# ratt-ru/pfb-clean

Hardware: AMD Instinct MI355X
Metric: PCG matvecs/sec (FFT-conv A^H A apply), 4k x 4k x 8-band cube (higher is better)
Workload: dtype f32; 1 GPU; 4096x4096x8-band cube PCG (hessian_psf + Tikhonov, M = x/sigmainv, tol=0, minit=maxit=20); nx_psf=8192, bands_per_gpu=8, parallelism=band-shard x1, allreduce_hook=False

## Files before the change

include/pfb_hip.h:

```cpp
#ifndef PFB_HIP_H
#define PFB_HIP_H

#include <stddef.h>
#include <stdint.h>

#ifdef __cplusplus
extern "C" {
#endif

#define PFB_ABI_VERSION 1

#define PFB_F32 0
#define PFB_F64 1

#define PFB_OK               0
#define PFB_ERR_INVALID     -1
#define PFB_ERR_UNSUPPORTED -2
#define PFB_ERR_HIP         -3
#define PFB_ERR_NONFINITE   -4
#define PFB_ERR_ALLOC       -5
#define PFB_ERR_COMM        -6

#define PFB_PCG_CONVERGED     0
#define PFB_PCG_MAXIT         1
// ... 22 lines not shown
                      const void* x, const void* beam, double wsum, double sigmainv,
                      void* out, const void* dot_with, double* dot_out, void* stream);

int pfb_psfconv_apply_dots(pfb_conv_plan* plan, int band0, int nb,
                           const void* x, const void* beam, double wsum, double sigmainv,
                           void* out, const void* dot_with, const void* dot_with2,
                           double* dots_out, void* stream);

int pfb_psfconv_apply_dots_bands(pfb_conv_plan* plan, int band0, int nb,
                                 const void* x, const void* beam, double wsum, double sigmainv,
                                 void* out, const void* dot_with, const void* dot_with2,
                                 double* dots_out, void* stream);

int    pfb_psfconv_plan_info(const pfb_conv_plan* plan, int* fast_path, int* vb,
                             size_t* workspace_bytes);

int pfb_psfconv_set_profiling(pfb_conv_plan* plan, int on);
int pfb_psfconv_get_profile(pfb_conv_plan* plan, double stage_ms[3], int* napply);

#define PFB_REDUCE_WS_DOUBLES 8192

int pfb_dot(int dtype, const void* a, const void* b, size_t n,
            double* out, double* ws, void* stream);
int pfb_norm_diff_sums(int dtype, const void* x, const void* xp, size_t n,
                       double* out, double* ws, void* stream);
int pfb_any_nonzero(int dtype, const void* a, size_t n, double* out, double* ws,
                    void* stream);
int pfb_axpby(int dtype, double a, const void* x, double b, void* y, size_t n,
              void* stream);

// ... 162 lines not shown
```

pfb_clean_amd/_lib.py:

```python
import ctypes as C
import os

_HERE = os.path.dirname(os.path.abspath(__file__))
LIB_PATH = os.environ.get('PFB_HIP_LIB') or os.path.join(_HERE, 'libpfb_hip.so')

PFB_F32, PFB_F64 = 0, 1
PFB_OK = 0
ERRORS = {-1: 'invalid argument', -2: 'unsupported size/dtype', -3: 'HIP runtime error',
          -4: 'non-finite value', -5: 'device allocation failed', -6: 'band-shard exchange failed'}
PCG_STATUS = {0: 'converged', 1: 'maxit', 2: 'zero-residual', 3: 'breakdown'}
REDUCE_WS_DOUBLES = 8192


PFB_ERR_INVALID = -1
PFB_ERR_UNSUPPORTED = -2
PFB_ERR_ALLOC = -5
PFB_ERR_COMM = -6


class PfbHipError(RuntimeError):
    def __init__(self, code, msg):
        super().__init__(f"libpfb_hip: {ERRORS.get(code, code)}: {msg}")
        self.code = code

# ... 12 lines not shown

_vp, _i, _d, _sz = C.c_void_p, C.c_int, C.c_double, C.c_size_t
SIGNATURES = {
    'pfb_abi_version': (_i, []),
    'pfb_last_error': (C.c_char_p, []),
    'pfb_psfconv_plan_create': (_i, [_i, _i, _i, _i, _i, _i, C.POINTER(_vp)]),
    'pfb_psfconv_plan_destroy': (_i, [_vp]),
    'pfb_psfconv_set_psfhat': (_i, [_vp, _vp, _vp]),
    'pfb_psfconv_apply': (_i, [_vp, _i, _i, _vp, _vp, _d, _d, _vp, _vp, _vp, _vp]),
    'pfb_psfconv_set_psf': (_i, [_vp, _vp, _vp, _vp]),
    'pfb_psfhat_regrid': (_i, [_i, _vp, _i, _i, _i, _i, _i, _i, _i, _vp, _vp]),
    'pfb_psfhat_from_psf': (_i, [_i, _vp, _i, _i, _i, _vp, _vp]),
    'pfb_psfconv_apply_dots': (_i, [_vp, _i, _i, _vp, _vp, _d, _d, _vp, _vp, _vp, _vp, _vp]),
    'pfb_psfconv_apply_dots_bands': (_i, [_vp, _i, _i, _vp, _vp, _d, _d, _vp, _vp, _vp, _vp, _vp]),
    'pfb_psfconv_plan_info': (_i, [_vp, C.POINTER(_i), C.POINTER(_i), C.POINTER(_sz)]),
    'pfb_psfconv_set_profiling': (_i, [_vp, _i]),
    'pfb_psfconv_get_profile': (_i, [_vp, C.POINTER(_d), C.POINTER(_i)]),
    'pfb_dot': (_i, [_i, _vp, _vp, _sz, _vp, _vp, _vp]),
    'pfb_norm_diff_sums': (_i, [_i, _vp, _vp, _sz, _vp, _vp, _vp]),
    'pfb_any_nonzero': (_i, [_i, _vp, _sz, _vp, _vp, _vp]),
    'pfb_axpby': (_i, [_i, _d, _vp, _d, _vp, _sz, _vp]),
    'pfb_pcg_work_bytes': (_sz, [_vp, _i]),
    'pfb_pcg_solve': (_i, [_vp, _i, _i, _vp, _vp, _vp, _vp, _d, _d, _d, _d, _i, _i, _i,
                           _vp, ALLREDUCE_FN, _vp, C.POINTER(PcgResult), _vp]),
    'pfb_pcg_bands_work_bytes': (_sz, [_vp, _i]),
    'pfb_pcg_solve_bands': (_i, [_vp, _i, _i, _vp, _vp, _vp, _vp, _d, _d, _d, _d, _i, _i, _i,
                                 _vp, C.POINTER(PcgResult), _vp]),
    'pfb_bandmix_dots': (_i, [_i, _vp, _vp, _i, _sz, _d, _vp, _vp, _vp, _vp, _vp, _vp]),
    'pfb_hessparam_work_bytes': (_sz, [_vp]),
    'pfb_hessparam_apply': (_i, [_vp, _vp, _vp, _vp, _d, _vp, _vp, _vp, _vp]),
# ... 78 lines not shown
```

pfb_clean_amd/csrc/cgvec.hip:

```cpp
#include "conv_plan.hpp"
#include "pcg_state.hpp"
#include <chrono>
#include <unistd.h>
#include <cstring>
#include <cstdlib>
#include <utility>
#include <vector>

namespace pfb {

constexpr int RED_MAX_GRID = 1024;

static inline int red_grid(size_t nvec) {
    size_t g = (nvec + RED_BLOCK - 1) / RED_BLOCK;
    g = (g + 3) / 4;
    if (g < 1) g = 1;
    if (g > (size_t)RED_MAX_GRID) g = RED_MAX_GRID;
    return (int)g;
}

template <typename T, int V>
__global__ void __launch_bounds__(RED_BLOCK)
k_dot(const T* __restrict__ a, const T* __restrict__ b, size_t nvec, double* __restrict__ ws) {
    double acc[1] = {0.0};
// ... 139 lines not shown
    for (size_t i = (size_t)blockIdx.x * blockDim.x + threadIdx.x; i < nvec;
         i += (size_t)gridDim.x * blockDim.x) {
        Pack<T, V> pp = ld<T, V>(p, i), pr = ld<T, V>(r, i);
#pragma unroll
        for (int e = 0; e < V; ++e) {
            const T y = mdiv > T(0) ? pr.e[e] / mdiv : pr.e[e];
            const T v = beta * pp.e[e] - y;
            pp.e[e] = v;
            acc[0] += (v != T(0)) ? 1.0 : 0.0;
        }
        st<T, V>(p, i, pp);
    }
    emit_partials<1>(acc, ws);
}

template <typename T, int V, int U, bool XNT, bool REV>
__global__ void __launch_bounds__(RED_BLOCK)
k_pcg_update_dir(const T* x, const T* r, T* __restrict__ p, const T* __restrict__ Ap, T* xn, T* rn,
                 const double* __restrict__ S, T mdiv, size_t nvs, int gps, double* __restrict__ ws) {
    const int s = blockIdx.x / gps, g = blockIdx.x - s * gps;
    const double* Sb = S + (size_t)s * SB;
    { const size_t off = (size_t)s * nvs * V; x += off; r += off; p += off; Ap += off; xn += off; rn += off; }
    double acc[4] = {0.0, 0.0, 0.0, 0.0};
    if (sys_live(Sb)) {
        const T alpha = (T)Sb[S_ALPHA];
        const T beta = (T)Sb[S_BETA];
        const size_t stride = (size_t)gps * blockDim.x;
        for (size_t i0 = (size_t)g * blockDim.x + threadIdx.x; i0 < nvs; i0 += U * stride) {
            Pack<T, V> px[U], pr[U], pp[U], pa[U];
#pragma unroll
            for (int u = 0; u < U; ++u) {
                const size_t ii = i0 + u * stride;
                const size_t i = REV ? nvs - 1 - ii : ii;
                if (ii < nvs) {
                    px[u] = XNT ? ld_nt<T, V>(x, i) : ld<T, V>(x, i);
                    pr[u] = ld<T, V>(r, i); pp[u] = ld<T, V>(p, i); pa[u] = ld<T, V>(Ap, i);
                }
            }
#pragma unroll
            for (int u = 0; u < U; ++u) {
                const size_t ii = i0 + u * stride;
                const size_t i = REV ? nvs - 1 - ii : ii;
                if (ii >= nvs) break;
                Pack<T, V> ox, orr;
#pragma unroll
                for (int e = 0; e < V; ++e) {
                    const T xnew = px[u].e[e] + alpha * pp[u].e[e];
                    const T rnew = pr[u].e[e] + alpha * pa[u].e[e];
                    const T y = mdiv > T(0) ? rnew / mdiv : rnew;
                    ox.e[e] = xnew;
                    orr.e[e] = rnew;
                    const double d = (double)xnew - (double)px[u].e[e];
                    acc[0] += (double)rnew * (double)y;
                    acc[1] += d * d;
                    acc[2] += (double)xnew * (double)xnew;
                    const T pn = beta * pp[u].e[e] - y;
                    pp[u].e[e] = pn;
                    acc[3] += (pn != T(0)) ? 1.0 : 0.0;
                }
                if constexpr (XNT) st_nt<T, V>(xn, i, ox); else st<T, V>(xn, i, ox);
                st<T, V>(rn, i, orr);
                st<T, V>(p, i, pp[u]);
            }
        }
    } else if (xn != x) {
        for (size_t i = (size_t)g * blockDim.x + threadIdx.x; i < nvs; i += (size_t)gps * blockDim.x) {
            st<T, V>(xn, i, ld<T, V>(x, i));
            st<T, V>(rn, i, ld<T, V>(r, i));
        }
    }
    emit_partials<4>(acc, ws);
}

__global__ void k_set_alpha(double* S) { S[S_ALPHA] = S[S_RHO] / S[S_PAP]; S[S_NBT] = 0.0; }
__global__ void k_scale_alpha(double* S) { S[S_ALPHA] *= 0.75; }
__global__ void k_set_beta(double* S) { S[S_BETA] = S[S_RHON] / S[S_RHO]; }
// ... 334 lines not shown
            return false;
        };
        int err;
        bool lookahead = n <= lookahead_max;
        if (const char* la = getenv("PFB_PCG_LOOKAHEAD")) lookahead = atoi(la) != 0;
        if (lookahead && plan->pcg_pin_n < nsys) {
            if (plan->pcg_pin) { PFB_HIP_CHECK(hipStreamSynchronize(st)); (void)hipHostFree(plan->pcg_pin); }
            plan->pcg_pin = nullptr;
            plan->pcg_pin_n = 0;
            PFB_HIP_CHECK(hipHostMalloc((void**)&plan->pcg_pin, sizeof(double) * 2 * nS, hipHostMallocDefault));
            plan->pcg_pin_n = nsys;
            for (int e = 0; e < 2; ++e)
                if (!plan->pcg_ev[e]) PFB_HIP_CHECK(hipEventCreateWithFlags(&plan->pcg_ev[e], hipEventDisableTiming));
        }
        const bool xnt = vec && n * sizeof(T) >= ((size_t)32 << 20);
        const double* seen = h.data();
        bool go = (1.0 > tol || 0 < minit) && 0 < maxit && any_live(seen);
        int khost = 0, slot = 0;
        bool pending_end = false, have_prev = false;
        int lo = 0, nl = nsys, gpl = update_grid(nvs, nsys);
        T *xc = x, *rc = r, *xn = xalt ? xalt : x, *rn = ralt ? ralt : r;
        auto narrow = [&](const double* hs) {
            int a = 0, z = nsys;
            while (a < z && !sys_live(hs + (size_t)a * SB)) ++a;
            while (z > a && !sys_live(hs + (size_t)(z - 1) * SB)) --z;
            if (z > a && (a != lo || z - a != nl)) { lo = a; nl = z - a; gpl = update_grid(nvs, nl); }
        };
        while (go) {
            const size_t off = (size_t)lo * ns;
            double* Sl = S + (size_t)lo * SB;
            typename PcgOp<T>::Partials c;
            if ((err = A.apply_partials(p, Ap, rc, lo, nl, &c)) != PFB_OK) return err;
            hipLaunchKernelGGL(k_iter_sums, dim3(nl), dim3(256), 0, st, c.cp, c.bs, c.qs, c.bst,
                               (const double*)ws, gpl, pending_end ? 1 : 0, Sl, mdiv_d, predict, hook ? 0 : 1);
            if (hook) {
                if ((err = sync.reduce(Sl + S_PAP, pending_end ? 7 : 4)) != PFB_OK) return err;
                if (pending_end) hipLaunchKernelGGL(k_iter_end_begin, dim3(1), dim3(1), 0, st, Sl, mdiv_d, predict);
                else hipLaunchKernelGGL(k_iter_begin, dim3(1), dim3(1), 0, st, Sl, mdiv_d, predict);
            }
            pending_end = false;
#define PFB_UPDATE(VV, XN)                                                                                     \
            hipLaunchKernelGGL((k_pcg_update_dir<T, VV, 2, XN, XN>), dim3(nl * gpl), dim3(RED_BLOCK), 0, st,   \
                               (const T*)xc + off, (const T*)rc + off, p + off, (const T*)Ap + off, xn + off,    \
                               rn + off, (const double*)Sl, mdiv, nvs, gpl, ws)
            if (xnt) PFB_UPDATE(V16<T>::N, true);
            else if (vec) PFB_UPDATE(V16<T>::N, false);
            else PFB_UPDATE(1, false);
#undef PFB_UPDATE
            std::swap(xc, xn);
            std::swap(rc, rn);
            if (khost + 1 < minit && khost + 1 < maxit) {
                pending_end = true;
            } else {
                if (hook) {
                    hipLaunchKernelGGL(k_iter_sums, dim3(nl), dim3(256), 0, st, (const double*)nullptr, 0, 0, 0,
                                       (const double*)ws, gpl, 1, Sl, mdiv_d, predict, 0);
                    if ((err = sync.reduce(Sl + S_RHON, 3)) != PFB_OK) return err;
                }
                hipLaunchKernelGGL(k_iter_end, dim3(nl), dim3(256), 0, st, hook ? nullptr : (const double*)ws, gpl, Sl);
            }
            PFB_HIP_CHECK(hipGetLastError());
            ++khost;
// ... 196 lines not shown
```

pfb_clean_amd/csrc/conv_plan.hpp:

```cpp
#pragma once
#include "common.hpp"
#include "fft_generic.hpp"

struct pfb_partial_layout {
    int slots, band_slots, q_stride, band_stride;
};

struct pfb_conv_plan {
    int nx, ny, P, Q, M;
    int nband, dtype;
    int VB, nvb;
    int fast;
    int long_lines;
    void* long_ws;
    size_t long_ws_bytes;
    pfb::FftFactors frow;
    pfb::FftFactors fcol;
    void* twP;
    void* twQ;
    void* psf_l;
    void* T;
    double* partials;
    size_t T_elems_per_band;
    size_t psf_elems_per_band;
    size_t workspace_bytes;
    int have_psf;
    int partials_per_band;
    pfb_partial_layout last;
    void* fast_tables;
    int prof_on, prof_n, prof_tick;
    hipEvent_t* prof_ev;
    double* pcg_pin;
    int pcg_pin_n;
    hipEvent_t pcg_ev[2];
};

namespace pfb {
inline size_t vec_bytes(const pfb_conv_plan* plan, int nb) {
    const size_t b = (size_t)nb * plan->nx * plan->ny * (plan->dtype == PFB_F32 ? 4 : 8);
    return (b + 255) & ~(size_t)255;
}
constexpr int PROF_MAX = 512;
inline void prof_mark(pfb_conv_plan* p, hipStream_t st, int k) {
    if (!p->prof_on) return;
// ... 23 lines not shown
```

pfb_clean_amd/csrc/fftconv.hip:

```cpp
#include "conv_plan.hpp"
#include "fft_long.hpp"
#include <algorithm>
#include <vector>
#include <cstring>
#include <cstdlib>

namespace pfb {

thread_local char g_err[512] = "";
void set_error(const char* fmt, ...) {
    va_list ap;
    va_start(ap, fmt);
    vsnprintf(g_err, sizeof(g_err), fmt, ap);
    va_end(ap);
}

struct ConvDims {
    int nx, ny, P, Q, M;
    size_t T_band, psf_band;
};

__device__ __forceinline__ size_t t_index(const ConvDims& d, int band, int i, int v) {
    return (size_t)band * d.T_band + (size_t)v * d.nx + i;
}
// ... 347 lines not shown
                            pfb_conv_plan** plan) {
    PFB_REQUIRE(plan != nullptr, PFB_ERR_INVALID, "plan_create: null plan pointer");
    *plan = nullptr;
    PFB_REQUIRE(dtype == PFB_F32 || dtype == PFB_F64, PFB_ERR_INVALID, "plan_create: bad dtype %d", dtype);
    PFB_REQUIRE(nx > 0 && ny > 0 && nband > 0, PFB_ERR_INVALID, "plan_create: non-positive size");
    PFB_REQUIRE(nx <= nx_psf && ny <= ny_psf, PFB_ERR_INVALID,
                "plan_create: image (%d,%d) larger than psf grid (%d,%d)", nx, ny, nx_psf, ny_psf);
    PFB_REQUIRE(ny_psf % 2 == 0, PFB_ERR_UNSUPPORTED,
                "plan_create: ny_psf=%d must be even (pfb's grid worker makes it so)", ny_psf);
    PFB_REQUIRE(factorable(nx_psf) && factorable(ny_psf / 2), PFB_ERR_UNSUPPORTED,
                "plan_create: (%d,%d) has a prime factor > 13", nx_psf, ny_psf);
    pfb_conv_plan* p = (pfb_conv_plan*)calloc(1, sizeof(pfb_conv_plan));
    PFB_REQUIRE(p != nullptr, PFB_ERR_ALLOC, "plan_create: host alloc failed");
    p->nx = nx; p->ny = ny; p->P = nx_psf; p->Q = ny_psf; p->M = ny_psf / 2;
    p->nband = nband; p->dtype = dtype;
    const size_t csz = dtype == PFB_F32 ? 8 : 16;
    p->fast = pow2_supported(p) ? 1 : 0;
    if (const char* e = getenv("PFB_FORCE_GENERIC")) { if (atoi(e)) p->fast = 0; }
    int vb = 1;
    p->partials_per_band = p->fast ? nx / pow2_rows_per_wg(p) : nx;
    if (p->fast) {
        vb = pow2_nvb(p);
        p->nvb = pow2_nblocks(p);
    } else {
        p->nvb = (p->M + 1 + vb - 1) / vb;
    }
    p->VB = vb;
    p->T_elems_per_band = (size_t)p->nvb * nx * vb;
    p->psf_elems_per_band = (size_t)p->nvb * p->P * vb;
    if (!plan_factors(p->M, &p->frow) || !plan_factors(p->P, &p->fcol)) {
// ... 40 lines not shown
    if (p->prof_ev) {
        for (int k = 0; k < 4 * PROF_MAX; ++k) (void)hipEventDestroy(p->prof_ev[k]);
        free(p->prof_ev);
    }
    if (p->pcg_pin) (void)hipHostFree(p->pcg_pin);
    for (int e = 0; e < 2; ++e) if (p->pcg_ev[e]) (void)hipEventDestroy(p->pcg_ev[e]);
    free(p);
    return PFB_OK;
}

int pfb_psfconv_plan_info(const pfb_conv_plan* p, int* fast_path, int* vb, size_t* workspace_bytes) {
    PFB_REQUIRE(p != nullptr, PFB_ERR_INVALID, "plan_info: null plan");
    if (fast_path) *fast_path = p->fast;
    if (vb) *vb = p->VB;
    if (workspace_bytes) *workspace_bytes = p->workspace_bytes;
    return PFB_OK;
}

int pfb_psfconv_set_profiling(pfb_conv_plan* p, int on) {
    PFB_REQUIRE(p != nullptr, PFB_ERR_INVALID, "set_profiling: null plan");
    if (on && !p->prof_ev) {
        p->prof_ev = (hipEvent_t*)calloc(4 * PROF_MAX, sizeof(hipEvent_t));
        PFB_REQUIRE(p->prof_ev != nullptr, PFB_ERR_ALLOC, "set_profiling: host alloc failed");
        for (int k = 0; k < 4 * PROF_MAX; ++k) PFB_HIP_CHECK(hipEventCreate(&p->prof_ev[k]));
    }
    p->prof_on = on > 0 ? on : 0;
    p->prof_n = 0;
    p->prof_tick = 0;
    return PFB_OK;
}
// ... 164 lines not shown
```

pfb_clean_amd/csrc/fftconv_pow2.hip:

```cpp
#include "conv_plan.hpp"
#include "fft_pow2.hpp"
#include <vector>
#include <cstdlib>
#include <type_traits>

#ifndef PFB_POW2_PART
#define PFB_POW2_PART 0
#endif
#define PFB_POW2_COL  (PFB_POW2_PART == 0 || PFB_POW2_PART == 2)
#define PFB_POW2_REST (PFB_POW2_PART == 0 || PFB_POW2_PART == 1)
#define PFB_POW2_MIX  (PFB_POW2_PART == 0 || PFB_POW2_PART == 3)
#define PFB_POW2_COLK  (PFB_POW2_COL || PFB_POW2_MIX)
#define PFB_POW2_RESTK (PFB_POW2_REST || PFB_POW2_MIX)

namespace pfb {

#ifndef PFB_STAMP
#define PFB_STAMP 0
#endif
#if PFB_STAMP
#define PFB_STAMP_ITS 4
#define PFB_STAMP_FIRST 2
static __device__ unsigned long long* g_stamp_buf = nullptr;
#define STAMP(KID, it, slot)                                                                              \
// ... 53 lines not shown
    return *reinterpret_cast<const Blk<T, NVB>*>(src);
}
template <typename T, int NVB>
__device__ __forceinline__ Blk<T, NVB> loadb_nt(const cplx<T>* src) {
    typedef float v4f __attribute__((ext_vector_type(4)));
    static_assert(sizeof(Blk<T, NVB>) == 16, "16-byte blocks");
    const v4f v = __builtin_nontemporal_load(reinterpret_cast<const v4f*>(src));
    Blk<T, NVB> b;
    __builtin_memcpy(&b, &v, 16);
    return b;
}

template <typename T, int NVB>
__device__ __forceinline__ void storeb(cplx<T>* dst, const Blk<T, NVB>& b) {
    *reinterpret_cast<Blk<T, NVB>*>(dst) = b;
}

template <typename P>
__device__ __forceinline__ P* opaque(P* p) {
    asm volatile("" : "+v"(p));
    return p;
}

__device__ __forceinline__ int launder(int v) {
    asm volatile("" : "+v"(v));
    return v;
}

template <typename T>
__device__ __forceinline__ cplx<T> root32(int k) {
// ... 741 lines not shown
    }
    __device__ __forceinline__ static int tile_row(int rg, int tiles_per_band) {
        constexpr int SH = 8 / G;
        if constexpr (SH > 1) {
            if (tiles_per_band % (8 * SH) == 0) {
                const int q = rg / (8 * SH), rem = rg % (8 * SH);
                rg = SH * (q * 8 + (rem & 7)) + (rem >> 3);
            }
        }
        return rg * G;
    }
};

template <typename T, int L, int PAR, typename Hook>
__device__ __forceinline__ void fwdp_post_lin(const cplx<T>* zr, const cplx<T>* ltm, cplx<T> wq1,
                                              cplx<T>* __restrict__ Tb, int nx, int i0, int rr, int bi, const Hook& hook);
template <typename T, int L, int PAR, typename Hook = NoPassHook>
__device__ __forceinline__ void fwdp_post(const cplx<T>* zr, const cplx<T>* ltm, cplx<T> wq1,
                                          cplx<T>* __restrict__ Tb, int nx, int i0, int rr, int bi,
                                          const Hook& hook = Hook()) {
    fwdp_post_lin<T, L, PAR, Hook>(zr, ltm, wq1, Tb, nx, i0, rr, bi, hook);
}

template <typename T, int L, int PAR, int K, int NREG, typename Hook>
__device__ __forceinline__ void post_steps_lin(const cplx<T>* const (&za)[FastCfg<T>::NVB], const cplx<T>* const (&zb)[FastCfg<T>::NVB],
                                               const cplx<T>* lw, cplx<T> wq1, cplx<T>* ub, size_t ustep, unsigned voff,
                                               bool first0, const Hook& hook) {
    using P = FwdP<T, L>;
    using F = typename P::F;
    constexpr int NVB = P::NVB, MS = NVB * P::BSTEP;
    if constexpr (K < NREG) {
        hook(PassIdx<K>{});
        Blk<T, NVB> o;
#pragma unroll
        for (int h = 0; h < NVB; ++h) {
            cplx<T> w;
            if constexpr (P::SMT) w = K == 0 ? lw[h] : lw[h] * root32<T>(P::KR * K);
            else w = lw[MS * K + h];
            if (PAR) w = w * wq1;
            const cplx<T> zv = za[h][F::cpad(MS * K)];
            cplx<T> zm = zb[h][F::cpad(MS * (NREG - 1 - K))];
            if constexpr (PAR == 0 && K == 0) { if (first0 && h == 0) zm = zv; }
            o.c[h] = T(0.5) * addrot<false>(addc(zv, zm), w * subc(zv, zm));
        }
        storeb<T, NVB>(ub + (size_t)K * ustep + voff, o);
        __builtin_amdgcn_sched_barrier(0);
        post_steps_lin<T, L, PAR, K + 1, NREG, Hook>(za, zb, lw, wq1, ub, ustep, voff, first0, hook);
    }
}

template <typename T, int L, int PAR, typename Hook>
__device__ __forceinline__ void fwdp_post_lin(const cplx<T>* zr, const cplx<T>* ltm, cplx<T> wq1,
                                              cplx<T>* __restrict__ Tb, int nx, int i0, int rr, int bi,
                                              const Hook& hook) {
    using P = FwdP<T, L>;
    using F = typename P::F;
    constexpr int NVB = P::NVB, BS = P::BSTEP, MS = NVB * BS;
    constexpr int NBP = PAR ? P::NBO : P::NBE;
    constexpr int NIT = (NBP + BS - 1) / BS;
    constexpr int NREG = PAR ? NIT : NIT - 1;
    static_assert(MS % 16 == 0, "a step keeps the padding phase");
    static_assert(PAR ? (NBP == NIT * BS) : (NBP == (NIT - 1) * BS + 1), "block counts of the two sweeps");
    cplx<T>* ub = Tb + (size_t)(PAR ? P::NBE : 0) * nx * NVB;
    const size_t ustep = (size_t)BS * nx * NVB;
    const unsigned voff = ((unsigned)bi * (unsigned)nx + (unsigned)(i0 + rr)) * NVB;
    const int m0 = NVB * bi;
    const cplx<T>* za[NVB];
    const cplx<T>* zb[NVB];
#pragma unroll
    for (int h = 0; h < NVB; ++h) {
        za[h] = zr + F::pad(m0 + h);
        zb[h] = zr + F::pad(L - PAR - (m0 + h) - MS * (NREG - 1));
    }
    post_steps_lin<T, L, PAR, 0, NREG, Hook>(za, zb, ltm + m0, wq1, ub, ustep, voff, bi == 0, hook);
    if constexpr (PAR == 0) {
        hook(PassIdx<NREG>{});
        const cplx<T> z0 = zr[F::pad(0)];
        Blk<T, NVB> o;
        o.c[0] = T(0.5) * addrot<false>(addc(z0, z0), cplx<T>(T(-1), T(0)) * subc(z0, z0));
#pragma unroll
        for (int h = 1; h < NVB; ++h) o.c[h] = cplx<T>(0, 0);
        storeb<T, NVB>(ub + (size_t)(NBP - 1) * nx * NVB + (unsigned)(i0 + rr) * NVB, o);
        __builtin_amdgcn_sched_barrier(0);
    }
}

template <typename T, int L, bool BEAM>
__global__ void __launch_bounds__((FwdP<T, L>::NT))
k_row_fwd_pow2q(const T* __restrict__ x, const T* __restrict__ beam, cplx<T>* __restrict__ Tw, const cplx<T>* __restrict__ twM,
                const cplx<T>* __restrict__ ptwc, FastDims d, int band0, int tiles_per_band, int ntiles,
                cplx<T> wq1) {
    using P = FwdP<T, L>;
    constexpr int E = P::EOK;
    using F = RegFft<T, L, E, false, 0, true, false>;
    constexpr int TPB = F::TPB, G = P::G, NT = P::NT, NP = F::NPASS;
    using V2 = typename vec2<T>::type;
    extern __shared__ __attribute__((aligned(16))) char smem[];
    cplx<T>* ltw = reinterpret_cast<cplx<T>*>(smem);
    cplx<T>* ltm = ltw + P::PTWP;
    cplx<T>* lds0 = ltm + P::NTM;
    int vb = blockIdx.x;
    if (vb >= ntiles) return;
    for (int k = threadIdx.x; k < F::PTWC; k += NT) ltw[k] = ptwc[k];
    for (int k = threadIdx.x; k < P::NTM; k += NT) ltm[k] = twM[k];
    V2 xa[E], ba[BEAM ? E : 1];
    {
        const int bl = vb / tiles_per_band, i0 = P::tile_row(vb - bl * tiles_per_band, tiles_per_band);
        const int g = threadIdx.x / TPB, t = threadIdx.x % TPB;
        const size_t off = (size_t)bl * d.xband + (size_t)(i0 + g) * d.xpitch;
        const V2* xr = reinterpret_cast<const V2*>(x + off) + t;
#pragma unroll
        for (int j = 0; j < E; ++j) xa[j] = xr[TPB * j];
        if constexpr (BEAM) {
            const V2* br = reinterpret_cast<const V2*>(beam + off) + t;
#pragma unroll
            for (int j = 0; j < E; ++j) ba[j] = br[TPB * j];
        }
    }
    __syncthreads();
    for (int sit = 0;; ++sit) {
        STAMP(0, sit, 0);
        const int vbn = vb + (int)gridDim.x < ntiles ? vb + (int)gridDim.x : vb;
        const int bl = vb / tiles_per_band, i0 = P::tile_row(vb - bl * tiles_per_band, tiles_per_band);
        cplx<T>* Tb = Tw + (size_t)(band0 + bl) * d.T_band;
        cplx<T> vv[E];
        {
            const int tid = launder((int)threadIdx.x);
            const int g = tid / TPB, t = tid % TPB;
            cplx<T>* lds = lds0 + (size_t)g * P::STRIDE;
#pragma unroll
            for (int j = 0; j < E; ++j) {
                if constexpr (BEAM) { xa[j].x *= ba[j].x; xa[j].y *= ba[j].y; }
                vv[j] = cplx<T>(xa[j].x, xa[j].y);
            }
            STAMP(0, sit, 1);
            F::template run<false>(vv, lds, t, ltw);
            STAMP(0, sit, 2);
        }
        {
            const int tid = launder((int)threadIdx.x);
            const int g = tid / TPB, t = tid % TPB;
            __syncthreads();
            cplx<T>* wp = lds0 + (size_t)g * P::STRIDE + F::pad(t);
#pragma unroll
            for (int j = 0; j < E; ++j) wp[F::cpad(TPB * j)] = vv[j];
            __syncthreads();
        }
        STAMP(0, sit, 3);
        {
            const int tid = launder((int)threadIdx.x);
            fwdp_post<T, L, 0>(lds0 + (size_t)(tid % G) * P::STRIDE, ltm, wq1, Tb, d.nx, i0, tid % G, tid / G);
        }
        STAMP(0, sit, 4);
        {
            const int tid = launder((int)threadIdx.x);
            const int g = tid / TPB, t = tid % TPB;
            cplx<T>* lds = lds0 + (size_t)g * P::STRIDE;
#pragma unroll
            for (int j = 0; j < E; ++j) {
                vv[j] = cplx<T>(xa[j].x, xa[j].y) * P::tw_row(ltm, t, j);
                if ((j & 3) == 3) __builtin_amdgcn_sched_barrier(0);
            }
            const int bln = vbn / tiles_per_band, i0n = P::tile_row(vbn - bln * tiles_per_band, tiles_per_band);
            const size_t offn = (size_t)bln * d.xband + (size_t)(i0n + g) * d.xpitch;
            const V2* xr = reinterpret_cast<const V2*>(x + offn) + t;
            const V2* br = BEAM ? reinterpret_cast<const V2*>(beam + offn) + t : nullptr;
            F::template run<false>(vv, lds, t, ltw, [&](auto k) {
                constexpr int K = decltype(k)::value;
#pragma unroll
                for (int j = (K * E) / NP; j < ((K + 1) * E) / NP; ++j) {
                    xa[j] = xr[TPB * j];
                    if constexpr (BEAM) ba[j] = br[TPB * j];
                }
            });
            STAMP(0, sit, 5);
        }
        {
            const int tid = launder((int)threadIdx.x);
            const int g = tid / TPB, t = tid % TPB;
            cplx<T>* wp = lds0 + (size_t)g * P::STRIDE + F::pad(t);
            __syncthreads();
#pragma unroll
            for (int j = 0; j < E; ++j) wp[F::cpad(TPB * j)] = vv[j];
            __syncthreads();
            fwdp_post<T, L, 1>(lds0 + (size_t)(tid % G) * P::STRIDE, ltm, wq1, Tb, d.nx, i0, tid % G, tid / G);
            STAMP(0, sit, 6);
            __syncthreads();
        }
        STAMP(0, sit, 7);
        if (vbn == vb) break;
        vb = vbn;
    }
}

template <typename T, int L, int E, int PAR, typename PF>
__device__ __forceinline__ void row_inv_phase(PF&& after_loads_issued, const cplx<T>* __restrict__ Tb,
                                              const cplx<T>* __restrict__ twQ,
                                              const cplx<T>* __restrict__ ptw, cplx<T>* lds0,
                                              cplx<T>* lds, int nx, int i0, int t,
                                              cplx<T> (&vv)[E]) {
// ... 752 lines not shown
}
#endif

#if PFB_POW2_RESTK
template <typename T, int L> constexpr bool fwdp_ok() {
    if constexpr (odd_part(L) > 1) return false;
    else return FwdP<T, L>::OK;
}
template <typename T, int L> struct RowFwdK {
    using FP = FwdP<T, L>;
    static constexpr bool PERSISTENT = fwdp_ok<T, L>();
    static constexpr int E = [] { if constexpr (PERSISTENT) return FP::EOK; else return RowCfg<T, L, false>::E; }();
    static constexpr auto plain() { return k_row_fwd_pow2<T, L, E>; }
    template <typename Fn> static void reachable(Fn&& f) {
        if constexpr (PERSISTENT) {
            f(k_row_fwd_pow2q<T, L, false>, false);
            f(k_row_fwd_pow2q<T, L, true>, true);
        } else {
            f(plain(), false);
        }
    }
};

template <typename T, int L> struct RowInvK {
    static constexpr int E = RowCfg<T, L, true>::E, EP = InvPE<T, L>::E;
    using IP = InvP<T, L, EP>;
    static constexpr bool PERSISTENT = IP::OK;
    static constexpr bool PER_BAND = PERSISTENT && inv_pb_ok<T, L, EP>();
    static constexpr auto plain() { return k_row_inv_pow2<T, L, E>; }
    template <int MODE, bool PB, typename Fn> static void beam_pair(Fn&& f) {
        f(k_row_inv_pow2p<T, L, EP, MODE, false, PB>, MODE, false, PB);
        f(k_row_inv_pow2p<T, L, EP, MODE, true, PB>, MODE, true, PB);
    }
    template <typename Fn> static void persistent(Fn&& f) {
// ... 11 lines not shown
};

template <typename T, int L>
static int row_prepare(FastTables* ft) {
    using FK = RowFwdK<T, L>;
    using IK = RowInvK<T, L>;
    int rc;
    if constexpr (FK::PERSISTENT) rc = upload_ptwc<T, L, FK::E>(&ft->tab[PTWC_ROW_FWD]);
    else rc = upload_ptw<T, L, FK::E>(&ft->tab[PTW_ROW]);
    if (rc == PFB_OK) rc = upload_ptwc<T, L, IK::E>(&ft->tab[PTWC_ROW_INV]);
    if constexpr (IK::EP != IK::E) {
        if (rc == PFB_OK) rc = upload_ptwc<T, L, IK::EP>(&ft->tab[PTWC_ROW_INV_P]);
    } else {
        ft->tab[PTWC_ROW_INV_P] = ft->tab[PTWC_ROW_INV];
    }
    FK::reachable([&](auto* k, bool) { if (rc == PFB_OK) rc = set_lds_max(k); });
    IK::reachable([&](auto* k) { if (rc == PFB_OK) rc = set_lds_max(k); });
    return rc;
}

template <typename T>
static int prep_tables(pfb_conv_plan* p, FastTables* ft) {
    const int L = p->ny / 2;
    int rc = is_pow2(p->nx) ? pow2_col_prepare(p, ft) : pow2_mix_col_prepare(p, ft);
    if (rc != PFB_OK) return rc;
    if (!is_pow2(L)) rc = pow2_mix_row_prepare(p, ft);
    else if (!for_pow2_size(L, [&](auto l) { rc = row_prepare<T, l()>(ft); })) return PFB_ERR_UNSUPPORTED;
    if (rc != PFB_OK) return rc;
    return upload_table<T>(&ft->tab[TW_M], L, [&](cplx<T>* h) {
        const long double two_pi = 6.283185307179586476925286766559005768L;
        for (int n = 0; n < L; ++n) {
// ... 80 lines not shown
static cplx<T> wq1_of(const pfb_conv_plan* p) {
    const long double a = 6.283185307179586476925286766559005768L / (2.0L * (long double)p->ny);
    return cplx<T>((T)cosl(a), (T)(-sinl(a)));
}

template <typename T, int L>
static void launch_row_fwd(pfb_conv_plan* p, const FastTables* ft, void* Tbuf, int band0, int nb, const void* x,
                           const void* beam, size_t xpitch, size_t xband, hipStream_t st) {
    using K = RowFwdK<T, L>;
    const FastDims d = fast_dims(p, xpitch, xband);
    if constexpr (K::PERSISTENT) {
        using FP = typename K::FP;
        const int tiles_per_band = p->nx / FP::G, ntiles = tiles_per_band * nb;
        const int grid = ntiles < ft->num_cu * FP::WG_PER_CU ? ntiles : ft->num_cu * FP::WG_PER_CU;
        const cplx<T> wq1 = wq1_of<T>(p);
        K::reachable([&](auto* k, bool bm) {
            if (bm != (beam != nullptr)) return;
            hipLaunchKernelGGL(k, dim3(grid), dim3(FP::NT), FP::LDS, st, (const T*)x,
                               (const T*)beam, (cplx<T>*)Tbuf, (const cplx<T>*)ft->tab[TW_M],
                               (const cplx<T>*)ft->tab[PTWC_ROW_FWD], d, band0, tiles_per_band, ntiles, wq1);
        });
    } else {
        constexpr int E = K::E;
        using F = RegFft<T, L, E, RowCfg<T, L, false>::WAVE>;
        constexpr int G = row_groups<T, L, E, RowCfg<T, L, false>::GMAX>();
        static_assert(ROW_TILE_MAX % G == 0, "pow2_supported: the row tile divides nx");
        const size_t lds = sizeof(cplx<T>) * (size_t)G * (F::LDS_ELEMS + 4);
        hipLaunchKernelGGL(K::plain(), dim3(p->nx / G, nb), dim3(G * F::TPB), lds, st,
                           (const T*)x, (const T*)beam, (cplx<T>*)Tbuf, (const cplx<T>*)p->twQ,
                           (const cplx<T>*)ft->tab[TW_M], (const cplx<T>*)ft->tab[PTW_ROW], d, band0);
    }
}

template <typename T>
static int set_psf_t(pfb_conv_plan* p, const void* psf, void* psfhat_out, hipStream_t st) {
// ... 209 lines not shown
```

pfb_clean_amd/operators/psf.py:

```python
import ctypes as C
import threading

import numpy as np
import torch

from .. import _lib, _dev
from .._plan import NativePlan, PlanCache


def _pow2ceil(n):
    p = 1
    while p < n:
        p *= 2
    return p


NX_FAST_MAX = 8192
NY_FAST_MAX = {torch.float32: 16384, torch.float64: 8192}
LINE_MAX = {torch.float32: 10240, torch.float64: 5120}
MIX_ALL = {
    'nx': {torch.float32: (96, 6144), torch.float64: (96, 6144)},
    'ny': {torch.float32: (160, 12288), torch.float64: (160, 6144)},
}
MIX_OFFERED = {
# ... 191 lines not shown
                _lib.check(self._lib.pfb_psfconv_apply(
                    self._h, int(band0), int(nb), _dev.ptr(xs), _dev.ptr(bs),
                    float(wsum) if wsum is not None else 0.0, float(sigmainv), _dev.ptr(os_),
                    _dev.ptr(ds), _dev.ptr(dot_out), _dev.stream()))
                out3.copy_(os_[:, :self.nx, :self.ny])
            return out3[0] if squeeze else out3
        xs, bs, ds, os_ = x3, beam, dot_with, out3
        with self.lock:
            self._enter_stream()
            _lib.check(self._lib.pfb_psfconv_apply(
                self._h, int(band0), int(nb), _dev.ptr(xs), _dev.ptr(bs),
                float(wsum) if wsum is not None else 0.0, float(sigmainv), _dev.ptr(os_),
                _dev.ptr(ds), _dev.ptr(dot_out), _dev.stream()))
        return out3[0] if squeeze else out3

    def set_profiling(self, on):
        _lib.check(self._lib.pfb_psfconv_set_profiling(self._h, int(on)))

    def get_profile(self):
        ms = (C.c_double * 3)()
        n = C.c_int()
        _lib.check(self._lib.pfb_psfconv_get_profile(self._h, ms, C.byref(n)))
        return tuple(ms), n.value


_cache = PlanCache(8)


def _fingerprint(psfhat):
    if isinstance(psfhat, np.ndarray):
# ... 44 lines not shown
```

Baseline: 430.1 cube-matvecs/s.

## Add cache-budget policy using nontemporal loads/stores for streaming buffers

Adds a per-plan cache budget (default 192 MiB) and uses it to choose nontemporal loads and stores. In the persistent forward row-FFT kernel, input x is loaded nontemporally and the early tiles of the transposed buffer are stored nontemporally, so only the last tiles that fit the budget stay resident in the last-level cache for the next stage. In the PCG direction update, r and Ap are read and written nontemporally when the vector exceeds the budget. The aim is to cut cache thrashing and keep the most recently written data cached for the consumer stage, at the cost of extra kernel variants and a budget heuristic that may not match the real MI355X cache size.

```diff
diff --git a/include/pfb_hip.h b/include/pfb_hip.h
--- a/include/pfb_hip.h
+++ b/include/pfb_hip.h
@@ -60,6 +60,8 @@
 
 int    pfb_psfconv_plan_info(const pfb_conv_plan* plan, int* fast_path, int* vb,
                              size_t* workspace_bytes);
+
+int pfb_psfconv_set_cache_budget(pfb_conv_plan* plan, size_t bytes);
 
 int pfb_psfconv_set_profiling(pfb_conv_plan* plan, int on);
 int pfb_psfconv_get_profile(pfb_conv_plan* plan, double stage_ms[3], int* napply);
diff --git a/pfb_clean_amd/_lib.py b/pfb_clean_amd/_lib.py
--- a/pfb_clean_amd/_lib.py
+++ b/pfb_clean_amd/_lib.py
@@ -50,6 +50,7 @@
     'pfb_psfconv_apply_dots': (_i, [_vp, _i, _i, _vp, _vp, _d, _d, _vp, _vp, _vp, _vp, _vp]),
     'pfb_psfconv_apply_dots_bands': (_i, [_vp, _i, _i, _vp, _vp, _d, _d, _vp, _vp, _vp, _vp, _vp]),
     'pfb_psfconv_plan_info': (_i, [_vp, C.POINTER(_i), C.POINTER(_i), C.POINTER(_sz)]),
+    'pfb_psfconv_set_cache_budget': (_i, [_vp, _sz]),
     'pfb_psfconv_set_profiling': (_i, [_vp, _i]),
     'pfb_psfconv_get_profile': (_i, [_vp, C.POINTER(_d), C.POINTER(_i)]),
     'pfb_dot': (_i, [_i, _vp, _vp, _sz, _vp, _vp, _vp]),
diff --git a/pfb_clean_amd/csrc/cgvec.hip b/pfb_clean_amd/csrc/cgvec.hip
--- a/pfb_clean_amd/csrc/cgvec.hip
+++ b/pfb_clean_amd/csrc/cgvec.hip
@@ -177,7 +177,7 @@
     emit_partials<1>(acc, ws);
 }
 
-template <typename T, int V, int U, bool XNT, bool REV>
+template <typename T, int V, int U, bool XNT, bool REV, bool RNT>
 __global__ void __launch_bounds__(RED_BLOCK)
 k_pcg_update_dir(const T* x, const T* r, T* __restrict__ p, const T* __restrict__ Ap, T* xn, T* rn,
                  const double* __restrict__ S, T mdiv, size_t nvs, int gps, double* __restrict__ ws) {
@@ -197,7 +197,9 @@
                 const size_t i = REV ? nvs - 1 - ii : ii;
                 if (ii < nvs) {
                     px[u] = XNT ? ld_nt<T, V>(x, i) : ld<T, V>(x, i);
-                    pr[u] = ld<T, V>(r, i); pp[u] = ld<T, V>(p, i); pa[u] = ld<T, V>(Ap, i);
+                    pr[u] = RNT ? ld_nt<T, V>(r, i) : ld<T, V>(r, i);
+                    pp[u] = ld<T, V>(p, i);
+                    pa[u] = RNT ? ld_nt<T, V>(Ap, i) : ld<T, V>(Ap, i);
                 }
             }
 #pragma unroll
@@ -222,7 +224,7 @@
                     acc[3] += (pn != T(0)) ? 1.0 : 0.0;
                 }
                 if constexpr (XNT) st_nt<T, V>(xn, i, ox); else st<T, V>(xn, i, ox);
-                st<T, V>(rn, i, orr);
+                if constexpr (RNT) st_nt<T, V>(rn, i, orr); else st<T, V>(rn, i, orr);
                 st<T, V>(p, i, pp[u]);
             }
         }
@@ -587,6 +589,7 @@
                 if (!plan->pcg_ev[e]) PFB_HIP_CHECK(hipEventCreateWithFlags(&plan->pcg_ev[e], hipEventDisableTiming));
         }
         const bool xnt = vec && n * sizeof(T) >= ((size_t)32 << 20);
+        const bool rnt = xnt && plan->cache.engaged(n * sizeof(T));
         const double* seen = h.data();
         bool go = (1.0 > tol || 0 < minit) && 0 < maxit && any_live(seen);
         int khost = 0, slot = 0;
@@ -612,13 +615,14 @@
                 else hipLaunchKernelGGL(k_iter_begin, dim3(1), dim3(1), 0, st, Sl, mdiv_d, predict);
             }
             pending_end = false;
-#define PFB_UPDATE(VV, XN)                                                                                     \
-            hipLaunchKernelGGL((k_pcg_update_dir<T, VV, 2, XN, XN>), dim3(nl * gpl), dim3(RED_BLOCK), 0, st,   \
+#define PFB_UPDATE(VV, XN, RN)                                                                                 \
+            hipLaunchKernelGGL((k_pcg_update_dir<T, VV, 2, XN, XN, RN>), dim3(nl * gpl), dim3(RED_BLOCK), 0, st, \
                                (const T*)xc + off, (const T*)rc + off, p + off, (const T*)Ap + off, xn + off,    \
                                rn + off, (const double*)Sl, mdiv, nvs, gpl, ws)
-            if (xnt) PFB_UPDATE(V16<T>::N, true);
-            else if (vec) PFB_UPDATE(V16<T>::N, false);
-            else PFB_UPDATE(1, false);
+            if (rnt) PFB_UPDATE(V16<T>::N, true, true);
+            else if (xnt) PFB_UPDATE(V16<T>::N, true, false);
+            else if (vec) PFB_UPDATE(V16<T>::N, false, false);
+            else PFB_UPDATE(1, false, false);
 #undef PFB_UPDATE
             std::swap(xc, xn);
             std::swap(rc, rn);
diff --git a/pfb_clean_amd/csrc/conv_plan.hpp b/pfb_clean_amd/csrc/conv_plan.hpp
--- a/pfb_clean_amd/csrc/conv_plan.hpp
+++ b/pfb_clean_amd/csrc/conv_plan.hpp
@@ -5,6 +5,17 @@
 struct pfb_partial_layout {
     int slots, band_slots, q_stride, band_stride;
 };
+
+struct pfb_cache_policy {
+    size_t budget;
+    bool engaged(size_t stream_bytes) const { return stream_bytes > budget; }
+    int keep_from(int nitems, size_t bytes_kept_per_item, size_t stream_bytes) const {
+        if (!engaged(stream_bytes)) return 0;
+        const size_t keep = budget / bytes_kept_per_item;
+        return keep >= (size_t)nitems ? 0 : nitems - (int)keep;
+    }
+};
+constexpr size_t PFB_CACHE_BUDGET_DEFAULT = (size_t)192 << 20;
 
 struct pfb_conv_plan {
     int nx, ny, P, Q, M;
@@ -28,6 +39,7 @@
     int partials_per_band;
     pfb_partial_layout last;
     void* fast_tables;
+    pfb_cache_policy cache;
     int prof_on, prof_n, prof_tick;
     hipEvent_t* prof_ev;
     double* pcg_pin;
diff --git a/pfb_clean_amd/csrc/fftconv.hip b/pfb_clean_amd/csrc/fftconv.hip
--- a/pfb_clean_amd/csrc/fftconv.hip
+++ b/pfb_clean_amd/csrc/fftconv.hip
@@ -385,6 +385,7 @@
     PFB_REQUIRE(p != nullptr, PFB_ERR_ALLOC, "plan_create: host alloc failed");
     p->nx = nx; p->ny = ny; p->P = nx_psf; p->Q = ny_psf; p->M = ny_psf / 2;
     p->nband = nband; p->dtype = dtype;
+    p->cache.budget = PFB_CACHE_BUDGET_DEFAULT;
     const size_t csz = dtype == PFB_F32 ? 8 : 16;
     p->fast = pow2_supported(p) ? 1 : 0;
     if (const char* e = getenv("PFB_FORCE_GENERIC")) { if (atoi(e)) p->fast = 0; }
@@ -455,6 +456,12 @@
     if (fast_path) *fast_path = p->fast;
     if (vb) *vb = p->VB;
     if (workspace_bytes) *workspace_bytes = p->workspace_bytes;
+    return PFB_OK;
+}
+
+int pfb_psfconv_set_cache_budget(pfb_conv_plan* p, size_t bytes) {
+    PFB_REQUIRE(p != nullptr, PFB_ERR_INVALID, "set_cache_budget: null plan");
+    p->cache.budget = bytes;
     return PFB_OK;
 }
 
diff --git a/pfb_clean_amd/csrc/fftconv_pow2.hip b/pfb_clean_amd/csrc/fftconv_pow2.hip
--- a/pfb_clean_amd/csrc/fftconv_pow2.hip
+++ b/pfb_clean_amd/csrc/fftconv_pow2.hip
@@ -91,6 +91,18 @@
 template <typename T, int NVB>
 __device__ __forceinline__ void storeb(cplx<T>* dst, const Blk<T, NVB>& b) {
     *reinterpret_cast<Blk<T, NVB>*>(dst) = b;
+}
+template <typename T, int NVB>
+__device__ __forceinline__ void storeb(cplx<T>* dst, const Blk<T, NVB>& b, bool nt) {
+    typedef float v4f __attribute__((ext_vector_type(4)));
+    static_assert(sizeof(Blk<T, NVB>) == 16, "16-byte blocks");
+    if (nt) {
+        v4f v;
+        __builtin_memcpy(&v, &b, 16);
+        __builtin_nontemporal_store(v, reinterpret_cast<v4f*>(dst));
+    } else {
+        storeb<T, NVB>(dst, b);
+    }
 }
 
 template <typename P>
@@ -862,18 +874,19 @@
 
 template <typename T, int L, int PAR, typename Hook>
 __device__ __forceinline__ void fwdp_post_lin(const cplx<T>* zr, const cplx<T>* ltm, cplx<T> wq1,
-                                              cplx<T>* __restrict__ Tb, int nx, int i0, int rr, int bi, const Hook& hook);
+                                              cplx<T>* __restrict__ Tb, int nx, int i0, int rr, int bi, bool nt,
+                                              const Hook& hook);
 template <typename T, int L, int PAR, typename Hook = NoPassHook>
 __device__ __forceinline__ void fwdp_post(const cplx<T>* zr, const cplx<T>* ltm, cplx<T> wq1,
-                                          cplx<T>* __restrict__ Tb, int nx, int i0, int rr, int bi,
+                                          cplx<T>* __restrict__ Tb, int nx, int i0, int rr, int bi, bool nt,
                                           const Hook& hook = Hook()) {
-    fwdp_post_lin<T, L, PAR, Hook>(zr, ltm, wq1, Tb, nx, i0, rr, bi, hook);
+    fwdp_post_lin<T, L, PAR, Hook>(zr, ltm, wq1, Tb, nx, i0, rr, bi, nt, hook);
 }
 
 template <typename T, int L, int PAR, int K, int NREG, typename Hook>
 __device__ __forceinline__ void post_steps_lin(const cplx<T>* const (&za)[FastCfg<T>::NVB], const cplx<T>* const (&zb)[FastCfg<T>::NVB],
                                                const cplx<T>* lw, cplx<T> wq1, cplx<T>* ub, size_t ustep, unsigned voff,
-                                               bool first0, const Hook& hook) {
+                                               bool first0, bool nt, const Hook& hook) {
     using P = FwdP<T, L>;
     using F = typename P::F;
     constexpr int NVB = P::NVB, MS = NVB * P::BSTEP;
@@ -891,15 +904,15 @@
             if constexpr (PAR == 0 && K == 0) { if (first0 && h == 0) zm = zv; }
             o.c[h] = T(0.5) * addrot<false>(addc(zv, zm), w * subc(zv, zm));
         }
-        storeb<T, NVB>(ub + (size_t)K * ustep + voff, o);
+        storeb<T, NVB>(ub + (size_t)K * ustep + voff, o, nt);
         __builtin_amdgcn_sched_barrier(0);
-        post_steps_lin<T, L, PAR, K + 1, NREG, Hook>(za, zb, lw, wq1, ub, ustep, voff, first0, hook);
+        post_steps_lin<T, L, PAR, K + 1, NREG, Hook>(za, zb, lw, wq1, ub, ustep, voff, first0, nt, hook);
     }
 }
 
 template <typename T, int L, int PAR, typename Hook>
 __device__ __forceinline__ void fwdp_post_lin(const cplx<T>* zr, const cplx<T>* ltm, cplx<T> wq1,
-                                              cplx<T>* __restrict__ Tb, int nx, int i0, int rr, int bi,
+                                              cplx<T>* __restrict__ Tb, int nx, int i0, int rr, int bi, bool nt,
                                               const Hook& hook) {
     using P = FwdP<T, L>;
     using F = typename P::F;
@@ -920,7 +933,7 @@
         za[h] = zr + F::pad(m0 + h);
         zb[h] = zr + F::pad(L - PAR - (m0 + h) - MS * (NREG - 1));
     }
-    post_steps_lin<T, L, PAR, 0, NREG, Hook>(za, zb, ltm + m0, wq1, ub, ustep, voff, bi == 0, hook);
+    post_steps_lin<T, L, PAR, 0, NREG, Hook>(za, zb, ltm + m0, wq1, ub, ustep, voff, bi == 0, nt, hook);
     if constexpr (PAR == 0) {
         hook(PassIdx<NREG>{});
         const cplx<T> z0 = zr[F::pad(0)];
@@ -928,16 +941,16 @@
         o.c[0] = T(0.5) * addrot<false>(addc(z0, z0), cplx<T>(T(-1), T(0)) * subc(z0, z0));
 #pragma unroll
         for (int h = 1; h < NVB; ++h) o.c[h] = cplx<T>(0, 0);
-        storeb<T, NVB>(ub + (size_t)(NBP - 1) * nx * NVB + (unsigned)(i0 + rr) * NVB, o);
+        storeb<T, NVB>(ub + (size_t)(NBP - 1) * nx * NVB + (unsigned)(i0 + rr) * NVB, o, nt);
         __builtin_amdgcn_sched_barrier(0);
     }
 }
 
-template <typename T, int L, bool BEAM>
+template <typename T, int L, bool BEAM, bool XNT>
 __global__ void __launch_bounds__((FwdP<T, L>::NT))
 k_row_fwd_pow2q(const T* __restrict__ x, const T* __restrict__ beam, cplx<T>* __restrict__ Tw, const cplx<T>* __restrict__ twM,
                 const cplx<T>* __restrict__ ptwc, FastDims d, int band0, int tiles_per_band, int ntiles,
-                cplx<T> wq1) {
+                cplx<T> wq1, int keep_from) {
     using P = FwdP<T, L>;
     constexpr int E = P::EOK;
     using F = RegFft<T, L, E, false, 0, true, false>;
@@ -952,13 +965,24 @@
     for (int k = threadIdx.x; k < F::PTWC; k += NT) ltw[k] = ptwc[k];
     for (int k = threadIdx.x; k < P::NTM; k += NT) ltm[k] = twM[k];
     V2 xa[E], ba[BEAM ? E : 1];
+    auto ldx = [](const V2* q) -> V2 {
+        if constexpr (XNT) {
+            typedef T v2e __attribute__((ext_vector_type(2)));
+            const v2e v = __builtin_nontemporal_load(reinterpret_cast<const v2e*>(q));
+            V2 r;
+            r.x = v.x; r.y = v.y;
+            return r;
+        } else {
+            return *q;
+        }
+    };
     {
         const int bl = vb / tiles_per_band, i0 = P::tile_row(vb - bl * tiles_per_band, tiles_per_band);
         const int g = threadIdx.x / TPB, t = threadIdx.x % TPB;
         const size_t off = (size_t)bl * d.xband + (size_t)(i0 + g) * d.xpitch;
         const V2* xr = reinterpret_cast<const V2*>(x + off) + t;
 #pragma unroll
-        for (int j = 0; j < E; ++j) xa[j] = xr[TPB * j];
+        for (int j = 0; j < E; ++j) xa[j] = ldx(xr + TPB * j);
         if constexpr (BEAM) {
             const V2* br = reinterpret_cast<const V2*>(beam + off) + t;
 #pragma unroll
@@ -971,6 +995,7 @@
         const int vbn = vb + (int)gridDim.x < ntiles ? vb + (int)gridDim.x : vb;
         const int bl = vb / tiles_per_band, i0 = P::tile_row(vb - bl * tiles_per_band, tiles_per_band);
         cplx<T>* Tb = Tw + (size_t)(band0 + bl) * d.T_band;
+        const bool tnt = vb < keep_from;
         cplx<T> vv[E];
         {
             const int tid = launder((int)threadIdx.x);
@@ -997,7 +1022,7 @@
         STAMP(0, sit, 3);
         {
             const int tid = launder((int)threadIdx.x);
-            fwdp_post<T, L, 0>(lds0 + (size_t)(tid % G) * P::STRIDE, ltm, wq1, Tb, d.nx, i0, tid % G, tid / G);
+            fwdp_post<T, L, 0>(lds0 + (size_t)(tid % G) * P::STRIDE, ltm, wq1, Tb, d.nx, i0, tid % G, tid / G, tnt);
         }
         STAMP(0, sit, 4);
         {
@@ -1017,7 +1042,7 @@
                 constexpr int K = decltype(k)::value;
 #pragma unroll
                 for (int j = (K * E) / NP; j < ((K + 1) * E) / NP; ++j) {
-                    xa[j] = xr[TPB * j];
+                    xa[j] = ldx(xr + TPB * j);
                     if constexpr (BEAM) ba[j] = br[TPB * j];
                 }
             });
@@ -1031,7 +1056,7 @@
 #pragma unroll
             for (int j = 0; j < E; ++j) wp[F::cpad(TPB * j)] = vv[j];
             __syncthreads();
-            fwdp_post<T, L, 1>(lds0 + (size_t)(tid % G) * P::STRIDE, ltm, wq1, Tb, d.nx, i0, tid % G, tid / G);
+            fwdp_post<T, L, 1>(lds0 + (size_t)(tid % G) * P::STRIDE, ltm, wq1, Tb, d.nx, i0, tid % G, tid / G, tnt);
             STAMP(0, sit, 6);
             __syncthreads();
         }
@@ -1814,10 +1839,14 @@
     static constexpr auto plain() { return k_row_fwd_pow2<T, L, E>; }
     template <typename Fn> static void reachable(Fn&& f) {
         if constexpr (PERSISTENT) {
-            f(k_row_fwd_pow2q<T, L, false>, false);
-            f(k_row_fwd_pow2q<T, L, true>, true);
+            f(k_row_fwd_pow2q<T, L, false, false>, false, false);
+            f(k_row_fwd_pow2q<T, L, true, false>, true, false);
+            if constexpr (!FP::SMT) {
+                f(k_row_fwd_pow2q<T, L, false, true>, false, true);
+                f(k_row_fwd_pow2q<T, L, true, true>, true, true);
+            }
         } else {
-            f(plain(), false);
+            f(plain(), false, false);
         }
     }
 };
@@ -1859,7 +1888,7 @@
     } else {
         ft->tab[PTWC_ROW_INV_P] = ft->tab[PTWC_ROW_INV];
     }
-    FK::reachable([&](auto* k, bool) { if (rc == PFB_OK) rc = set_lds_max(k); });
+    FK::reachable([&](auto* k, bool, bool) { if (rc == PFB_OK) rc = set_lds_max(k); });
     IK::reachable([&](auto* k) { if (rc == PFB_OK) rc = set_lds_max(k); });
     return rc;
 }
@@ -1970,11 +1999,15 @@
         const int tiles_per_band = p->nx / FP::G, ntiles = tiles_per_band * nb;
         const int grid = ntiles < ft->num_cu * FP::WG_PER_CU ? ntiles : ft->num_cu * FP::WG_PER_CU;
         const cplx<T> wq1 = wq1_of<T>(p);
-        K::reachable([&](auto* k, bool bm) {
-            if (bm != (beam != nullptr)) return;
+        const size_t tile_bytes = sizeof(cplx<T>) * p->T_elems_per_band / tiles_per_band;
+        const size_t t_bytes = sizeof(cplx<T>) * p->T_elems_per_band * (size_t)nb;
+        const bool xnt = !FP::SMT && p->cache.engaged(t_bytes);
+        const int keep_from = FP::SMT ? 0 : p->cache.keep_from(ntiles, tile_bytes, t_bytes);
+        K::reachable([&](auto* k, bool bm, bool xn) {
+            if (bm != (beam != nullptr) || xn != xnt) return;
             hipLaunchKernelGGL(k, dim3(grid), dim3(FP::NT), FP::LDS, st, (const T*)x,
                                (const T*)beam, (cplx<T>*)Tbuf, (const cplx<T>*)ft->tab[TW_M],
-                               (const cplx<T>*)ft->tab[PTWC_ROW_FWD], d, band0, tiles_per_band, ntiles, wq1);
+                               (const cplx<T>*)ft->tab[PTWC_ROW_FWD], d, band0, tiles_per_band, ntiles, wq1, keep_from);
         });
     } else {
         constexpr int E = K::E;
diff --git a/pfb_clean_amd/operators/psf.py b/pfb_clean_amd/operators/psf.py
--- a/pfb_clean_amd/operators/psf.py
+++ b/pfb_clean_amd/operators/psf.py
@@ -229,6 +229,9 @@
                 _dev.ptr(ds), _dev.ptr(dot_out), _dev.stream()))
         return out3[0] if squeeze else out3
 
+    def set_cache_budget(self, nbytes):
+        _lib.check(self._lib.pfb_psfconv_set_cache_budget(self._h, min(int(nbytes), 2 ** 64 - 1)))
+
     def set_profiling(self, on):
         _lib.check(self._lib.pfb_psfconv_set_profiling(self._h, int(on)))
 
```

After: 438.1 cube-matvecs/s, median of 6. 1.02x the previous value.
